# davelailai/DS-GCN

Hardware: AMD Instinct MI355X
Metric: clips/sec fwd+bwd, DS-STGCN NTU-60 3x64x25x2 (higher is better)
Workload: dtype f32; 1 GPU; DS-STGCN configs/dsstgcn/ntu60_xsub_3dkp/j.py (DSSTGCN_model.py kwargs), 64 clips/GPU of 3x64x25x2, 60 classes, train-mode BN, CE loss, fwd+bwd+grad all-reduce+SGD-nesterov per step; clips_per_gpu=64, global_batch=64, parallelism=dp1

## Files before the change

ds-gcn_amd/csrc/fuseout.hip:

```cpp
#include "common.h"
#include "dropout.h"
#include "dsgcn_jobs.h"

namespace {

__global__ __launch_bounds__(64) void k_fuse_out_fwd(const float* __restrict__ x1, const float* __restrict__ s1,
                                                     const float* __restrict__ h1, const float* __restrict__ x2,
                                                     const float* __restrict__ s2, const float* __restrict__ h2,
                                                     int relu, float* __restrict__ out, float* __restrict__ xbar, int C,
                                                     int T, int V, int vec, int ld, float* __restrict__ out_s2,
                                                     float* __restrict__ pmean, DropArgs dr) {
  extern __shared__ __attribute__((aligned(16))) float lds[];
  const int lane = threadIdx.x;
  const long plane = blockIdx.x;
  const int c = (int)(plane % C);
  const int L = T * V;
  const bool drop = dr.thresh != 0;
  const unsigned long long dstep = (drop && dr.step) ? (unsigned long long)*dr.step : 0ull;
  const float a1 = s1 ? s1[c] : 1.f, b1 = s1 ? h1[c] : 0.f;
  const float a2 = s2 ? s2[c] : 1.f, b2 = s2 ? h2[c] : 0.f;
  const float* p1 = x1 + (size_t)plane * L;
  const float* p2 = x2 ? x2 + (size_t)plane * L : nullptr;
  float* po = out ? out + (size_t)plane * L : nullptr;
  float psum = 0.f;
  if (vec) {
    const int L4 = L >> 2;
    const f32x4* q1 = reinterpret_cast<const f32x4*>(p1);
    const f32x4* q2 = reinterpret_cast<const f32x4*>(p2);
    f32x4* qo = reinterpret_cast<f32x4*>(po);
    f32x4* ql = reinterpret_cast<f32x4*>(lds);
#pragma unroll 4
    for (int i = lane; i < L4; i += 64) {
      f32x4 v = q1[i];
      v.x = fmaf(v.x, a1, b1); v.y = fmaf(v.y, a1, b1); v.z = fmaf(v.z, a1, b1); v.w = fmaf(v.w, a1, b1);
      if (relu & 2) { v.x = fmaxf(v.x, 0.f); v.y = fmaxf(v.y, 0.f); v.z = fmaxf(v.z, 0.f); v.w = fmaxf(v.w, 0.f); }
      if (drop) {
        unsigned rw[4];
        drop_words(dr, dstep, (unsigned long long)plane * L4 + i, rw);
        v.x *= rw[0] >= dr.thresh ? dr.inv : 0.f; v.y *= rw[1] >= dr.thresh ? dr.inv : 0.f;
        v.z *= rw[2] >= dr.thresh ? dr.inv : 0.f; v.w *= rw[3] >= dr.thresh ? dr.inv : 0.f;
      }
      if (p2) {
        const f32x4 r = q2[i];
        v.x += fmaf(r.x, a2, b2); v.y += fmaf(r.y, a2, b2); v.z += fmaf(r.z, a2, b2); v.w += fmaf(r.w, a2, b2);
      }
      if (relu & 1) { v.x = fmaxf(v.x, 0.f); v.y = fmaxf(v.y, 0.f); v.z = fmaxf(v.z, 0.f); v.w = fmaxf(v.w, 0.f); }
      if (po) qo[i] = v;
      psum += (v.x + v.y) + (v.z + v.w);
      if (xbar || out_s2) ql[i] = v;
    }
  } else {
    for (int i = lane; i < L; i += 64) {
      float v = fmaf(p1[i], a1, b1);
      if (relu & 2) v = fmaxf(v, 0.f);
      if (drop) v *= drop_mult(dr, dstep, (unsigned long long)plane * L + i);
      if (p2) v += fmaf(p2[i], a2, b2);
      if (relu & 1) v = fmaxf(v, 0.f);
      if (po) po[i] = v;
      psum += v;
      if (xbar || out_s2) lds[i] = v;
    }
  }
  if (pmean) {
    psum = wave_sum(psum);
    if (lane == 0) pmean[plane] = psum / (float)L;
  }
  if (xbar || out_s2) wave_lds_sync();
  if (out_s2) {
    const int T2 = (T + 1) >> 1, L2 = T2 * V;
    float* ps = out_s2 + (size_t)plane * L2;
    const float invV = 1.f / (float)V;
    if ((L2 & 3) == 0) {
      f32x4* q4 = reinterpret_cast<f32x4*>(ps);
      for (int i = lane; i < (L2 >> 2); i += 64) {
        int t, v;
        divmod_small(4 * i, V, invV, t, v);
        float r[4];
#pragma unroll
        for (int k = 0; k < 4; ++k) {
          r[k] = lds[2 * t * V + v];
          if (++v == V) { v = 0; ++t; }
        }
// ... 59 lines not shown
    float g = s3 == 3 ? gpl : (pg ? pg[i] : 0.f);
    if (pg2) g += pg2[i];
    if (pg3) {
      if (s3 == 2) { if (!(t & 1)) g += pg3[(t >> 1) * V + v]; }
      else g += pg3[i];
    }
    g += dxb[v];
    if ((relu & 1) && !(pre > 0.f)) g = 0.f;
    const float g1 = (((relu & 2) && !(pre1 > 0.f)) ? 0.f : g) * dm;
    o1[i] = g1 * a1;
    if (o2) o2[i] = g * a2;
    u0 = fmaf(g1, xa, u0);
    u1 += g;
    u2 = fmaf(g, xb, u2);
    u3 += g1;
    v += step;
    t += tstep;
    if (v >= V) { v -= V; ++t; }
  }
  if (part) {
    u0 = wave_sum(u0);
    u1 = wave_sum(u1);
    u2 = wave_sum(u2);
    u3 = wave_sum(u3);
    if (lane == 0) {
      part[(size_t)plane * 4 + 0] = u0;
      part[(size_t)plane * 4 + 1] = u1;
      part[(size_t)plane * 4 + 2] = u2;
      part[(size_t)plane * 4 + 3] = u3;
    }
  }
}

template <int NG, bool S3, bool X2>
__global__ __launch_bounds__(64) void k_fuse_out_bwd4(const float* __restrict__ x1, const float* __restrict__ s1,
                                                      const float* __restrict__ h1, const float* __restrict__ x2,
                                                      const float* __restrict__ s2, const float* __restrict__ h2,
                                                      int relu, const float* __restrict__ dout,
                                                      const float* __restrict__ dout2, const float* __restrict__ dout3,
                                                      const float* __restrict__ dxbar, float* __restrict__ dx1,
                                                      float* __restrict__ dx2, float* __restrict__ part, int C, int T,
                                                      int V, int ld, DropArgs dr) {
  __shared__ float dxb[32];
  const int lane = threadIdx.x;
  const long plane = blockIdx.x;
  const int c = (int)(plane % C);
  const int L = T * V, L4 = L >> 2;
  const bool drop = dr.thresh != 0;
  const unsigned long long dstep = (drop && dr.step) ? (unsigned long long)*dr.step : 0ull;
  const float a1 = s1 ? s1[c] : 1.f, b1 = s1 ? h1[c] : 0.f;
  const float a2 = s2 ? s2[c] : 1.f, b2 = s2 ? h2[c] : 0.f;
  if (lane < V) dxb[lane] = dxbar ? dxbar[(size_t)plane * ld + lane] / (float)T : 0.f;
  wave_lds_sync();
  const f32x4* __restrict__ p1 = reinterpret_cast<const f32x4*>(x1 + (size_t)plane * L);
  const f32x4* __restrict__ p2 = X2 ? reinterpret_cast<const f32x4*>(x2 + (size_t)plane * L) : nullptr;
  const f32x4* __restrict__ pg = NG >= 1 ? reinterpret_cast<const f32x4*>(dout + (size_t)plane * L) : nullptr;
  const float gplane = NG == 0 ? dout[plane] / (float)L : 0.f;
  const f32x4* __restrict__ pg2 = NG >= 2 ? reinterpret_cast<const f32x4*>(dout2 + (size_t)plane * L) : nullptr;
  const f32x4* __restrict__ pg3 = (NG >= 3 && !S3) ? reinterpret_cast<const f32x4*>(dout3 + (size_t)plane * L) : nullptr;
  const float* __restrict__ ps3 = S3 ? dout3 + (size_t)plane * (((T + 1) >> 1) * V) : nullptr;
  f32x4* __restrict__ o1 = reinterpret_cast<f32x4*>(dx1 + (size_t)plane * L);
  f32x4* __restrict__ o2 = X2 ? reinterpret_cast<f32x4*>(dx2 + (size_t)plane * L) : nullptr;
  const float invV = 1.f / (float)V;
  float u0 = 0.f, u1 = 0.f, u2 = 0.f, u3 = 0.f;
  for (int i = lane; i < L4; i += 64) {
    const f32x4 xa = p1[i];
    f32x4 xb = {0.f, 0.f, 0.f, 0.f}, g = {gplane, gplane, gplane, gplane};
    if constexpr (NG >= 1) g = pg[i];
    if constexpr (X2) xb = p2[i];
    if constexpr (NG >= 2) { const f32x4 w = pg2[i]; g.x += w.x; g.y += w.y; g.z += w.z; g.w += w.w; }
    if constexpr (NG >= 3 && !S3) { const f32x4 w = pg3[i]; g.x += w.x; g.y += w.y; g.z += w.z; g.w += w.w; }
    int t, v;
    divmod_small(4 * i, V, invV, t, v);
    f32x4 r1, r2;
    float dm[4] = {1.f, 1.f, 1.f, 1.f};
    if (drop) {
      unsigned rw[4];
      drop_words(dr, dstep, (unsigned long long)plane * L4 + i, rw);
#pragma unroll
      for (int k = 0; k < 4; ++k) dm[k] = rw[k] >= dr.thresh ? dr.inv : 0.f;
    }
#pragma unroll
    for (int k = 0; k < 4; ++k) {
      float gg = g[k];
      if constexpr (S3) { if (!(t & 1)) gg += ps3[(t >> 1) * V + v]; }
      gg += dxb[v];
      const float pre1 = fmaf(xa[k], a1, b1);
      float pre = ((relu & 2) ? fmaxf(pre1, 0.f) : pre1) * dm[k];
      if constexpr (X2) pre += fmaf(xb[k], a2, b2);
      if ((relu & 1) && !(pre > 0.f)) gg = 0.f;
      const float g1 = (((relu & 2) && !(pre1 > 0.f)) ? 0.f : gg) * dm[k];
      r1[k] = g1 * a1;
      r2[k] = gg * a2;
      u0 = fmaf(g1, xa[k], u0);
      u1 += gg;
      u2 = fmaf(gg, xb[k], u2);
      u3 += g1;
      if (++v == V) { v = 0; ++t; }
    }
    o1[i] = r1;
    if constexpr (X2) o2[i] = r2;
  }
  if (part) {
    u0 = wave_sum(u0);
    u1 = wave_sum(u1);
    u2 = wave_sum(u2);
    u3 = wave_sum(u3);
    if (lane == 0) {
      part[(size_t)plane * 4 + 0] = u0;
      part[(size_t)plane * 4 + 1] = u1;
      part[(size_t)plane * 4 + 2] = u2;
      part[(size_t)plane * 4 + 3] = u3;
    }
  }
}

int g_fo_vec = 1;

}

namespace {

DropArgs drop_args(const dsgcn_dropout* d) {
  DropArgs a = {};
  if (d && d->p > 0.f) {
    a.step = d->step; a.seed = d->seed; a.call = d->call;
    double t = (double)d->p * 4294967296.0;
    a.thresh = t >= 4294967295.0 ? 4294967295u : (t < 1.0 ? 1u : (unsigned)t);
    a.inv = 1.f / (1.f - d->p);
  }
  return a;
}

__global__ __launch_bounds__(256) void k_dropout_mask(float* __restrict__ mask, long numel, DropArgs dr) {
  const unsigned long long step = dr.step ? (unsigned long long)*dr.step : 0ull;
  for (long e = (long)blockIdx.x * 256 + threadIdx.x; e < numel; e += (long)gridDim.x * 256)
    mask[e] = dr.thresh ? drop_mult(dr, step, (unsigned long long)e) : 1.f;
}

}

extern "C" {

int dsgcn_fuse_out_fwd_drop(const float* x1, const float* s1, const float* h1, const float* x2, const float* s2,
                            const float* h2, int relu, float* out, float* out_s2, float* xbar, float* pmean, int n, int C,
                            int T, int V, int xbar_ld, const dsgcn_dropout* d, void* stream) {
  if (!x1 || (!out && !pmean) || n <= 0 || C <= 0 || T <= 0 || V <= 0 || V > 32 || (s1 && !h1) || (s2 && !h2)) return DSGCN_EINVAL;
  if ((out_s2 || xbar) && !out) return DSGCN_EINVAL;
  if (xbar && (xbar_ld < V || xbar_ld > 64)) return DSGCN_EINVAL;
  if (d && !(d->p >= 0.f && d->p < 1.f)) return DSGCN_EINVAL;
  const int vec = ((T * V) % 4 == 0) ? 1 : 0;
  const size_t lds = (xbar || out_s2) ? (size_t)T * V * sizeof(float) : 0;
  if (lds > 64 * 1024) return DSGCN_EUNSUPPORTED;
  hipLaunchKernelGGL(k_fuse_out_fwd, dim3((unsigned)((long)n * C)), dim3(64), lds, (hipStream_t)stream, x1, s1, h1, x2,
                     s2, h2, relu, out, xbar, C, T, V, vec, xbar ? xbar_ld : V, out_s2, pmean, drop_args(d));
  DSGCN_LAUNCH_CHECK();
  return 0;
}

int dsgcn_fuse_out_fwd(const float* x1, const float* s1, const float* h1, const float* x2, const float* s2,
                       const float* h2, int relu, float* out, float* xbar, int n, int C, int T, int V, int xbar_ld,
                       void* stream) {
  if (!out) return DSGCN_EINVAL;
  return dsgcn_fuse_out_fwd_drop(x1, s1, h1, x2, s2, h2, relu, out, nullptr, xbar, nullptr, n, C, T, V, xbar_ld, nullptr, stream);
}

int dsgcn_fuse_out_bwd_drop(const float* x1, const float* s1, const float* h1, const float* x2, const float* s2,
                            const float* h2, int relu, const float* dout, const float* dout2, const float* dout3,
                            int stride3, const float* dxbar, float* dx1, float* dx2, float* part, int n, int C, int T, int V,
                            int xbar_ld, const dsgcn_dropout* d, void* stream) {
  if (!x1 || !dx1 || n <= 0 || C <= 0 || T <= 0 || V <= 0 || V > 32 || (x2 && !dx2)) return DSGCN_EINVAL;
  if (dxbar && xbar_ld < V) return DSGCN_EINVAL;
  if ((dout2 || dout3) && !dout) return DSGCN_EINVAL;
  if (stride3 < 1 || stride3 > 3 || (stride3 == 3 && (!dout || dout2 || dout3 || dxbar))) return DSGCN_EINVAL;
  if (d && !(d->p >= 0.f && d->p < 1.f)) return DSGCN_EINVAL;
  const DropArgs dr = drop_args(d);
  const dim3 grid((unsigned)((long)n * C)), blk(64);
  hipStream_t st = (hipStream_t)stream;
  if (stride3 == 3) {
    if ((T * V) % 4 == 0) {
      if (x2)
        hipLaunchKernelGGL((k_fuse_out_bwd4<0, false, true>), grid, blk, 0, st, x1, s1, h1, x2, s2, h2, relu, dout,
                           (const float*)nullptr, (const float*)nullptr, (const float*)nullptr, dx1, dx2, part, C, T, V, V, dr);
      else
        hipLaunchKernelGGL((k_fuse_out_bwd4<0, false, false>), grid, blk, 0, st, x1, s1, h1, x2, s2, h2, relu, dout,
                           (const float*)nullptr, (const float*)nullptr, (const float*)nullptr, dx1, dx2, part, C, T, V, V, dr);
    } else {
      hipLaunchKernelGGL(k_fuse_out_bwd, grid, blk, 0, st, x1, s1, h1, x2, s2, h2, relu, dout, (const float*)nullptr,
                         (const float*)nullptr, (const float*)nullptr, dx1, dx2, part, C, T, V, V, 3, dr);
    }
    DSGCN_LAUNCH_CHECK();
    return 0;
  }
  if (g_fo_vec && dout && (T * V) % 4 == 0 && !(dout3 && !dout2 && stride3 == 1)) {
    const int ng = dout3 && stride3 == 1 ? 3 : (dout2 ? 2 : 1);
    const bool s3 = dout3 && stride3 == 2;
#define FO4(NGV, S3V, X2V) hipLaunchKernelGGL((k_fuse_out_bwd4<NGV, S3V, X2V>), grid, blk, 0, st, x1, s1, h1, x2, s2, h2, relu, \
                                              dout, dout2, dout3, dxbar, dx1, dx2, part, C, T, V, xbar_ld, dr)
    if (x2) {
      if (s3) { if (ng == 2) FO4(2, true, true); else FO4(1, true, true); }
      else if (ng == 3) FO4(3, false, true);
      else if (ng == 2) FO4(2, false, true);
      else FO4(1, false, true);
    } else {
      if (s3) { if (ng == 2) FO4(2, true, false); else FO4(1, true, false); }
      else if (ng == 3) FO4(3, false, false);
      else if (ng == 2) FO4(2, false, false);
      else FO4(1, false, false);
    }
#undef FO4
    DSGCN_LAUNCH_CHECK();
    return 0;
  }
  hipLaunchKernelGGL(k_fuse_out_bwd, grid, blk, 0, st, x1, s1, h1, x2, s2, h2, relu, dout, dout2, dout3, dxbar, dx1, dx2,
                     part, C, T, V, xbar_ld, stride3, dr);
  DSGCN_LAUNCH_CHECK();
  return 0;
}

int dsgcn_dropout_mask(float* mask, long numel, const dsgcn_dropout* d, void* stream) {
  if (!mask || numel <= 0 || (d && !(d->p >= 0.f && d->p < 1.f))) return DSGCN_EINVAL;
  const long blocks = (numel + 255) / 256;
  hipLaunchKernelGGL(k_dropout_mask, dim3((unsigned)(blocks > 4096 ? 4096 : blocks)), dim3(256), 0, (hipStream_t)stream, mask,
                     numel, drop_args(d));
  DSGCN_LAUNCH_CHECK();
  return 0;
}

#ifdef DSGCN_LAB
int dsgcn_fuse_out_tuning(int key, int value) {
  if (key != 0) return DSGCN_EINVAL;
  g_fo_vec = value;
  return 0;
}
#endif

int dsgcn_fuse_out_bwd(const float* x1, const float* s1, const float* h1, const float* x2, const float* s2,
                       const float* h2, int relu, const float* dout, const float* dxbar, float* dx1, float* dx2,
                       float* part, int n, int C, int T, int V, int xbar_ld, void* stream) {
  return dsgcn_fuse_out_bwd_drop(x1, s1, h1, x2, s2, h2, relu, dout, nullptr, nullptr, 1, dxbar, dx1, dx2, part, n, C, T, V,
                                 xbar_ld, nullptr, stream);
}

}

namespace {
__global__ __launch_bounds__(256) void k_pack(const float* const* __restrict__ src, const long* __restrict__ off,
                                              const int* __restrict__ numel, float* __restrict__ dst) {
  const int i = blockIdx.x;
  const float* __restrict__ s = src[i];
  float* __restrict__ d = dst + off[i];
  const int n = numel[i];
// ... 67 lines not shown
```

ds-gcn_amd/kernels.py:

```python
import contextlib
import sys

_active = None


def ops():
    return _active if _active is not None else sys.modules[__name__]


@contextlib.contextmanager
def use_ops(namespace):
    global _active
    prev = _active
    _active = namespace
    try:
        yield namespace
    finally:
        _active = prev


NAME = 'hip'

import torch

# ... 2350 lines not shown
FUSE_OUT_LDS_BYTES = 64 * 1024


def prestrided_fits(T, V):
    return T * V * 4 <= FUSE_OUT_LDS_BYTES


_drop_state = {'call': 0, 'step': {}, 'used': False}


def _dropout_record(p, device):
    st = _drop_state
    if device not in st['step']:
        st['step'][device] = torch.zeros((), dtype=torch.int64, device=device)
    st['call'] = (st['call'] + 1) & 0x7fffffff
    st['used'] = True
    step = st['step'][device]
    return native.Dropout(step.data_ptr(), int(torch.initial_seed()) & 0xffffffffffffffff, st['call'], float(p)), step


def dropout_step_advance():
    if _drop_state['used']:
        for step in _drop_state['step'].values():
            step.add_(1)


def dropout_mask(numel, rec):
    dev = next(iter(_drop_state['step']))
    out = torch.empty(numel, device=dev, dtype=torch.float32)
    native.check(native.lib().dsgcn_dropout_mask(_ptr(out), numel, _ct.byref(rec), _stream()), 'dsgcn_dropout_mask')
    return out


class _FuseOut(torch.autograd.Function):

    @staticmethod
    def forward(ctx, x1, s1, h1, x2, s2, h2, relu, xbar_ld, tee, dropout=0.0):
        _require_cuda(x1)
        x1, s1, h1, x2, s2, h2 = [_f32c(t) for t in (x1, s1, h1, x2, s2, h2)]
        n, C, T, V = x1.shape
        if x2 is not None and x2.shape != x1.shape:
            raise ValueError(f'fuse_out: the two terms differ in shape: {tuple(x1.shape)} vs {tuple(x2.shape)}')
        out = torch.empty_like(x1)
        out_s2 = torch.empty((n, C, (T + 1) // 2, V), device=x1.device, dtype=torch.float32) if tee == 2 else None
        xbar = torch.empty((n, C, xbar_ld), device=x1.device, dtype=torch.float32) if xbar_ld else None
        ctx.drop = _dropout_record(dropout, x1.device) if dropout > 0 else None
        rc = native.lib().dsgcn_fuse_out_fwd_drop(_ptr(x1), _ptr(s1), _ptr(h1), _ptr(x2), _ptr(s2), _ptr(h2), int(relu),
                                                  _ptr(out), _ptr(out_s2), _ptr(xbar), None, n, C, T, V, int(xbar_ld),
                                                  _ct.byref(ctx.drop[0]) if ctx.drop else None, _stream())
        native.check(rc, 'dsgcn_fuse_out_fwd_drop')
        ctx.save_for_backward(x1, s1, h1, x2, s2, h2)
        ctx.relu = int(relu)
        ctx.xbar_ld = int(xbar_ld)
        ctx.tee = int(tee)
        ctx.bn1, ctx.bn2 = _bn_of(s1), _bn_of(s2)
        ctx.set_materialize_grads(False)
        if tee == 2:
            return out, out.view_as(out), out_s2, xbar
        if tee:
            return out, out.view_as(out), out.view_as(out), xbar
        return out, None, None, xbar

    @staticmethod
    def backward(ctx, dout, dout2, dout3, dxbar):
        x1, s1, h1, x2, s2, h2 = ctx.saved_tensors
        n, C, T, V = x1.shape
        stride3 = 1
        for g, frames in ((dout, T), (dout2, T), (dout3, (T + 1) // 2 if ctx.tee == 2 else T)):
            if g is not None and tuple(g.shape) != (n, C, frames, V):
                raise ValueError(f'fuse_out backward: gradient of shape {tuple(g.shape)}, expected {(n, C, frames, V)}')
        if ctx.tee == 2:
            d3 = _f32c(dout3)
            full = [_f32c(g) for g in (dout, dout2) if g is not None]
            if d3 is not None and not full:
                full = [torch.zeros_like(x1)]
            douts = full + [None] * (2 - len(full)) + [d3]
            stride3 = 2 if d3 is not None else 1
        else:
            douts = [_f32c(g) for g in (dout, dout2, dout3) if g is not None]
            douts += [None] * (3 - len(douts))
        dxbar = _f32c(dxbar)
        dx1 = torch.empty_like(x1)
        dx2 = torch.empty_like(x2) if x2 is not None else None
        need_part = s1 is not None or s2 is not None
        part = torch.empty((n, C, 4), device=x1.device, dtype=torch.float32) if need_part else None
        rc = native.lib().dsgcn_fuse_out_bwd_drop(_ptr(x1), _ptr(s1), _ptr(h1), _ptr(x2), _ptr(s2), _ptr(h2), ctx.relu,
                                                  _ptr(douts[0]), _ptr(douts[1]), _ptr(douts[2]), stride3, _ptr(dxbar),
                                                  _ptr(dx1), _ptr(dx2), _ptr(part), n, C, T, V, ctx.xbar_ld or V,
                                                  _ct.byref(ctx.drop[0]) if ctx.drop else None, _stream())
        native.check(rc, 'dsgcn_fuse_out_bwd_drop')
        (ds1, dh1, ds2, dh2), _ = _affine_tail(part, 4, [(s1, ctx.bn1, 0, 3), (s2, ctx.bn2, 2, 1)])
        return dx1, ds1, dh1, dx2, ds2, dh2, None, None, None, None


class _FuseOutPool(torch.autograd.Function):

    @staticmethod
    def forward(ctx, x1, s1, h1, x2, s2, h2, relu, dropout=0.0):
        _require_cuda(x1)
        x1, s1, h1, x2, s2, h2 = [_f32c(t) for t in (x1, s1, h1, x2, s2, h2)]
        n, C, T, V = x1.shape
        if x2 is not None and x2.shape != x1.shape:
            raise ValueError(f'fuse_out_pool: the two terms differ in shape: {tuple(x1.shape)} vs {tuple(x2.shape)}')
        pm = torch.empty((n, C), device=x1.device, dtype=torch.float32)
        ctx.drop = _dropout_record(dropout, x1.device) if dropout > 0 else None
        rc = native.lib().dsgcn_fuse_out_fwd_drop(_ptr(x1), _ptr(s1), _ptr(h1), _ptr(x2), _ptr(s2), _ptr(h2), int(relu),
                                                  None, None, None, _ptr(pm), n, C, T, V, V,
                                                  _ct.byref(ctx.drop[0]) if ctx.drop else None, _stream())
        native.check(rc, 'dsgcn_fuse_out_fwd_drop')
        ctx.save_for_backward(x1, s1, h1, x2, s2, h2)
        ctx.relu = int(relu)
        ctx.bn1, ctx.bn2 = _bn_of(s1), _bn_of(s2)
        return pm

    @staticmethod
    def backward(ctx, dpm):
        x1, s1, h1, x2, s2, h2 = ctx.saved_tensors
        n, C, T, V = x1.shape
        dpm = _f32c(dpm)
        dx1 = torch.empty_like(x1)
        dx2 = torch.empty_like(x2) if x2 is not None else None
        need_part = s1 is not None or s2 is not None
        part = torch.empty((n, C, 4), device=x1.device, dtype=torch.float32) if need_part else None
# ... 164 lines not shown
```

ds-gcn_amd/native.py:

```python
import ctypes
import glob
import os
import subprocess

_HERE = os.path.dirname(os.path.abspath(__file__))
CSRC = os.path.join(_HERE, 'csrc')
LIB_DIR = os.path.join(_HERE, 'lib')
LIB_PATH = os.path.join(LIB_DIR, 'libdsgcn.so')
LAB_LIB_PATH = os.path.join(LIB_DIR, 'libdsgcn_lab.so')
INCLUDE = os.path.join(os.path.dirname(_HERE), 'include')

_lib = None
_lab = None
INITIAL_MATMUL_PRECISION = 0

c_f = ctypes.c_void_p
c_i = ctypes.c_void_p
c_int = ctypes.c_int
c_st = ctypes.c_void_p

SIGNATURES = {
    'dsgcn_version': [],
    'dsgcn_set_matmul_precision': [c_int],
    'dsgcn_get_matmul_precision': [],
# ... 73 lines not shown
    'dsgcn_ctr_affine_bwd': [ctypes.c_void_p, c_f, c_int, c_f, ctypes.c_void_p, c_f] + [c_int] * 4 + [c_st],
    'dsgcn_edge_select_fwd': [c_f, c_i, c_f] + [c_int] * 4 + [c_st],
    'dsgcn_edge_select_bwd': [c_f, c_i, c_f] + [c_int] * 4 + [c_st],
    'dsgcn_plane_stats': [c_f, c_f, ctypes.c_long, c_int, c_st],
    'dsgcn_typedconv_fwd': [c_f, c_f, c_f, c_i, c_int, c_f] + [c_int] * 7 + [c_st],
    'dsgcn_typedconv_dgrad': [c_f, c_f, c_i, c_int, c_f] + [c_int] * 7 + [c_st],
    'dsgcn_typedconv_wgrad_rows': [c_int] * 4,
    'dsgcn_typedconv_wgrad': [c_f, c_f, c_i, c_int, c_f] + [c_int] * 7 + [c_st],
    'dsgcn_add3': [c_f, c_f, c_f, c_f, ctypes.c_long, c_st],
    'dsgcn_pack': [c_f, c_f, c_f, c_int, c_f, c_st],
    'dsgcn_pack_fill': [c_f, c_f, c_f, c_int, c_f, c_st],
    'dsgcn_colsum_multi_host': [ctypes.c_void_p, c_int, c_st],
    'dsgcn_fuse_out_fwd': [c_f] * 6 + [c_int] + [c_f] * 2 + [c_int] * 5 + [c_st],
    'dsgcn_fuse_out_bwd': [c_f] * 6 + [c_int] + [c_f] * 5 + [c_int] * 5 + [c_st],
    'dsgcn_dwcausal_fwd': [c_f, c_f, c_f, c_i, c_f] + [c_int] * 6 + [c_st],
    'dsgcn_dwcausal_bwd': [c_f, c_f, c_i, c_f, c_f, c_f] + [c_int] * 6 + [c_st],
    'dsgcn_gate_fwd': [c_f, c_f, c_int, c_f, c_f] + [c_int] * 5 + [c_st],
    'dsgcn_gate_bwd': [c_f, c_f, c_int, c_f, c_f, c_int, c_f, c_f] + [c_int] * 4 + [c_st],
    'dsgcn_skeleton_prep': [ctypes.c_void_p] * 11 + [c_int] * 10 + [c_st],
    'dsgcn_skeleton_prep_streams': [ctypes.c_void_p] * 10 + [ctypes.POINTER(ctypes.c_void_p)] + [c_int] * 10 + [c_st],
    'dsgcn_dynadj_partial_stride': [c_int, c_int, c_int],
    'dsgcn_dynadj_supported': [c_int] * 6,
    'dsgcn_dynadj_fwd': [c_f] * 6 + [c_i, c_i, c_f] + [c_int] * 6 + [c_st],
    'dsgcn_dynadj_bwd': [c_f] * 5 + [c_i, c_i] + [c_f] * 4 + [c_int] * 7 + [c_st],
    'dsgcn_pwconv_group_ok': [c_int] * 5,
    'dsgcn_pwconv_fwd_group': [ctypes.c_void_p] * 3 + [c_int] + [ctypes.c_void_p] * 2 + [c_int] * 6 + [c_st],
    'dsgcn_pwconv_dgrad_group': [ctypes.c_void_p] * 3 + [c_int] + [ctypes.c_void_p] * 4 + [c_int] * 6 + [c_st],
    'dsgcn_pwconv_wgrad_group': [ctypes.c_void_p] * 3 + [c_int] + [ctypes.c_void_p] * 3 + [c_int] * 7 + [c_st],
    'dsgcn_pwconv_wgrad_jobs': [c_f] * 6 + [c_int] + [c_f] * 8 + [c_int] * 8 + [ctypes.c_void_p, c_int, c_st],
    'dsgcn_tms_split_wgrad_jobs': [c_f] * 4 + [c_int] + [c_f] * 2 + [c_int] * 6 + [c_i] * 4 + [ctypes.c_void_p, ctypes.c_void_p, c_int, c_int, ctypes.c_void_p, c_int, c_st],
    'dsgcn_fuse_out_fwd_drop': [c_f] * 6 + [c_int] + [c_f] * 4 + [c_int] * 5 + [ctypes.c_void_p, c_st],
    'dsgcn_fuse_out_bwd_drop': [c_f] * 6 + [c_int] + [c_f] * 3 + [c_int] + [c_f] * 4 + [c_int] * 5 + [ctypes.c_void_p, c_st],
    'dsgcn_dropout_mask': [c_f, ctypes.c_long, ctypes.c_void_p, c_st],
    'dsgcn_bn_finalize_multi': [ctypes.c_void_p, c_int, c_st],
    'dsgcn_bn_coef_rows_multi': [ctypes.c_void_p, c_int, c_st],
    'dsgcn_dyntyped_select_fwd': [c_f, c_i, c_f] + [c_int] * 5 + [c_st],
    'dsgcn_dyntyped_select_bwd': [c_f, c_i, c_f] + [c_int] * 5 + [c_st],
    'dsgcn_dyntyped_partial_stride': [c_int] * 4,
    'dsgcn_dyntyped_fwd': [c_f] * 6 + [c_i, c_f] + [c_int] * 5 + [c_st],
    'dsgcn_dyntyped_bwd': [c_f] * 5 + [c_i] + [c_f] * 5 + [c_int] * 6 + [c_st],
    'dsgcn_dynflag_partial_stride': [c_int] * 4,
    'dsgcn_dynflag_fwd': [c_f] * 8 + [c_i, c_i, c_f] + [c_int] * 7 + [c_st],
    'dsgcn_dynflag_bwd': [c_f] * 7 + [c_i, c_i] + [c_f] * 5 + [c_int] * 8 + [c_st],
    'dsgcn_dynplain_partial_stride': [c_int] * 2,
    'dsgcn_dynplain_fwd': [c_f] * 5 + [c_int] * 5 + [c_st],
    'dsgcn_dynplain_bwd': [c_f] * 6 + [c_int] * 6 + [c_st],
    'dsgcn_dynadj_fwd_jobs': [c_f] * 6 + [c_i, c_i, c_f] + [c_int] * 6 + [ctypes.c_void_p, c_int, c_st],
    'dsgcn_dynadj_bwd_jobs': [c_f] * 5 + [c_i, c_i] + [c_f] * 4 + [c_int] * 7 + [ctypes.c_void_p, c_int, c_st],
    'dsgcn_head_loss_fwd': [c_f, c_f, c_f, c_i] + [c_int] * 4 + [ctypes.c_float] + [c_f] * 6 + [c_st],
    'dsgcn_head_loss_bwd': [c_f, c_f, c_f, c_i, c_f] + [c_int] * 4 + [ctypes.c_float] + [c_f] * 3 + [c_st],
    'dsgcn_head_target_fwd': [c_f] * 4 + [ctypes.c_void_p] + [c_int] * 5 + [ctypes.c_float] + [c_f] * 7 + [c_st],
    'dsgcn_head_target_bwd': [c_f] * 5 + [c_int] * 4 + [ctypes.c_float] + [c_f] * 3 + [c_st],
    'dsgcn_head_test_fwd': [c_f, c_f, c_f] + [c_int] * 6 + [c_f, c_f, c_st],
    'dsgcn_head_ensemble_fwd': [ctypes.POINTER(ctypes.c_void_p)] * 3 + [c_f] + [c_int] * 7 + [c_f, c_f, c_st],
    'dsgcn_feat_ext_fwd': [c_f, c_f, c_f] + [c_int] * 8 + [c_f, ctypes.c_void_p, c_st],
    'dsgcn_data_bn_fwd': [c_f] * 10 + [c_int] * 7 + [ctypes.c_float, ctypes.c_float, c_st],
    'dsgcn_data_bn_bwd': [c_f] * 6 + [c_int] * 6 + [c_st],
    'dsgcn_sgd_step': [c_f, c_f, c_f, c_f, ctypes.c_float, ctypes.c_float, c_int, ctypes.c_longlong, c_st],
    'dsgcn_grad_norm_rows': [ctypes.c_longlong],
    'dsgcn_grad_norm_partials': [c_f, ctypes.c_longlong, c_int, ctypes.c_void_p, c_st],
    'dsgcn_sgd_step_clip': [c_f, c_f, c_f, c_f, ctypes.c_void_p, c_int, c_int, ctypes.c_float, c_f, ctypes.c_float,
                            ctypes.c_float, c_int, ctypes.c_longlong, c_st],
    'dsgcn_grad_accum': [c_f, c_f, ctypes.c_longlong, c_st],
    'dsgcn_grad_accum_finish': [c_f, c_f, c_f, ctypes.c_longlong, c_st],
    'dsgcn_optim_chunks': [ctypes.c_longlong],
    'dsgcn_optim_table': [ctypes.c_void_p, ctypes.c_void_p, c_int, ctypes.c_void_p, c_int, ctypes.c_longlong,
# ... 228 lines not shown
```

include/dsgcn.h:

```cpp
#ifndef DSGCN_H_
#define DSGCN_H_

#include <stddef.h>
#include "dsgcn_jobs.h"
#ifdef __cplusplus
extern "C" {
#endif

#define DSGCN_EINVAL (-1)
#define DSGCN_EUNSUPPORTED (-2)

int dsgcn_version(void);

int dsgcn_set_matmul_precision(int level);
int dsgcn_get_matmul_precision(void);
int dsgcn_pwconv_terms(int dir, int n, int Ci, int Co, int T, int V, int stride);
int dsgcn_tconv_terms(int dir, int n, int Ci, int Co, int T, int V, int KT, int stride);

int dsgcn_aggregate_fwd(const float* zp, const float* scale, const float* shift, int relu, const float* ahat,
                        float* y, int n, int KC, int T, int V, void* stream);

int dsgcn_aggregate_bwd_partial_rows(int n, int T, int V);
int dsgcn_aggregate_bwd(const float* zp, const float* scale, const float* shift, int relu, const float* ahat,
                        const float* dy, float* dzp, float* dahat, float* partial, int n, int KC, int T, int V,
// ... 26 lines not shown
int dsgcn_dyntyped_bwd(const float* x12, const float* pq, const float* be, const float* alpha, const float* beta,
                       const int* edge_type, const float* dahat, float* dd_ws, float* dx12, float* dpq, float* ppar,
                       int pstride, int n, int mid, int V, int E, int flags, void* stream);

int dsgcn_dynflag_partial_stride(int mid, int V, int E, int flags);
int dsgcn_dynflag_fwd(const float* proj, const float* pq, const float* be, const float* wa, const float* ba,
                      const float* A, const float* alpha, const float* beta, const int* node_type, const int* edge_type,
                      float* ahat, int n, int mid, int V, int ld, int P, int E, int flags, void* stream);
int dsgcn_dynflag_bwd(const float* proj, const float* pq, const float* be, const float* wa, const float* ba,
                      const float* alpha, const float* beta, const int* node_type, const int* edge_type,
                      const float* dahat, float* dd_ws, float* dproj, float* dpq, float* ppar, int pstride, int n,
                      int mid, int V, int ld, int P, int E, int flags, void* stream);

int dsgcn_dynplain_partial_stride(int K, int V);
int dsgcn_dynplain_fwd(const float* proj, const float* A, const float* alpha, const float* beta, float* ahat, int n, int K,
                       int mid, int V, int ld, void* stream);
int dsgcn_dynplain_bwd(const float* proj, const float* alpha, const float* beta, const float* dahat, float* dproj,
                       float* ppar, int pstride, int n, int K, int mid, int V, int ld, void* stream);

int dsgcn_fuse_out_fwd(const float* x1, const float* s1, const float* h1, const float* x2, const float* s2,
                       const float* h2, int relu, float* out, float* xbar, int n, int C, int T, int V, int xbar_ld,
                       void* stream);
int dsgcn_fuse_out_bwd(const float* x1, const float* s1, const float* h1, const float* x2, const float* s2,
                       const float* h2, int relu, const float* dout, const float* dxbar, float* dx1, float* dx2,
                       float* part, int n, int C, int T, int V, int xbar_ld, void* stream);
int dsgcn_fuse_out_fwd_drop(const float* x1, const float* s1, const float* h1, const float* x2, const float* s2,
                            const float* h2, int relu, float* out, float* out_s2, float* xbar, float* pmean, int n, int C,
                            int T, int V, int xbar_ld, const dsgcn_dropout* d, void* stream);
int dsgcn_fuse_out_bwd_drop(const float* x1, const float* s1, const float* h1, const float* x2, const float* s2,
                            const float* h2, int relu, const float* dout, const float* dout2, const float* dout3,
                            int stride3, const float* dxbar, float* dx1, float* dx2, float* part, int n, int C, int T, int V,
                            int xbar_ld, const dsgcn_dropout* d, void* stream);
int dsgcn_dropout_mask(float* mask, long numel, const dsgcn_dropout* d, void* stream);

size_t dsgcn_tconv_ws_bytes(int n, int Ci, int Co, int T, int V, int KT, int stride);
int dsgcn_tconv_wsplit(const float* w, int Ci, int Co, int KT, void* ws, void* stream);
int dsgcn_tconv_wsplit_multi(const dsgcn_tsplit_job* jobs, int njobs, void* stream);
int dsgcn_tconv_rows(int which, int n, int Ci, int Co, int T, int V, int KT, int stride);
int dsgcn_tconv_fwd(const float* x1, const float* s1, const float* h1, const float* x2, const float* s2, const float* h2,
                    int relu, const void* ws, const float* bias, float* z, float* partial, int n, int Ci, int Co, int T,
                    int V, int KT, int stride, void* stream);
int dsgcn_tconv_dgrad(const float* x1, const float* s1, const float* h1, const float* x2, const float* s2,
                      const float* h2, int relu, const void* ws, const float* z, const float* gz, const float* A0,
                      const float* B0, float* dx1, float* dx2, float* ipart, int n, int Ci, int Co, int T, int V, int KT,
                      int stride, void* stream);

int dsgcn_tconv_wgrad_splits(int n, int Ci, int Co, int T, int V, int KT, int stride);
int dsgcn_tconv_wgrad(const float* x1, const float* s1, const float* h1, const float* x2, const float* s2,
                      const float* h2, int relu, const float* z, const float* gz, const float* A0, const float* B0,
                      float* dwp, float* dbp, int pstride, int n, int Ci, int Co, int T, int V, int KT, int stride,
                      void* stream);

int dsgcn_branch_act_fwd(const float* z, const float* zaug, const float* scale, const float* shift, int n_act,
                         float* h, int n, int C, int T, int V, void* stream);
int dsgcn_branch_act_bwd(const float* z, const float* zaug, const float* scale, const float* shift, int n_act,
                         const float* dh, float* dz, float* dzaug, float* part, int n, int C, int T, int V,
                         void* stream);
int dsgcn_tapconv_fwd(const float* h, float* o, int n, int Cin, int Cout, int T, int V1, int stride, int KT, int nbr,
                      const int* type, const int* ci0, const int* co0, const int* cin, const int* cout, const int* dil,
                      const float* const* w, const float* const* b, void* stream);
int dsgcn_tapconv_dgrad(const float* h, const float* go, float* dh, int n, int Cin, int Cout, int T, int V1, int stride,
                        int KT, int nbr, const int* type, const int* ci0, const int* co0, const int* cin,
                        const int* cout, const int* dil, const float* const* w, void* stream);
int dsgcn_tapconv_wgrad_splits(int n, int Cin, int Cout, int T, int V1, int stride, int KT, int nbr, const int* type,
                               const int* cin, const int* cout, const int* dil);
int dsgcn_tapconv_wgrad(const float* h, const float* go, int n, int Cin, int Cout, int T, int V1, int stride, int KT,
// ... 274 lines not shown
```

Measured before the change: 6089 clips/s.

## Save a packed ReLU bitmask in fuse-out forward instead of reloading residual input

When the fused output has a residual term with no affine and a final ReLU, the forward kernel now packs the sign of each output element into a 1-bit mask. Backward reads that mask rather than the full float residual tensor x2 to recompute the ReLU gate, which cuts backward memory traffic for that kernel. The cost is an extra mask write plus wave shuffles in forward, and a small separate mask allocation. Keeping x2 saved for autograd does not by itself save memory. The path is on by default and can be disabled with an environment variable.

```diff
diff --git a/ds-gcn_amd/csrc/fuseout.hip b/ds-gcn_amd/csrc/fuseout.hip
--- a/ds-gcn_amd/csrc/fuseout.hip
+++ b/ds-gcn_amd/csrc/fuseout.hip
@@ -9,7 +9,8 @@
                                                      const float* __restrict__ s2, const float* __restrict__ h2,
                                                      int relu, float* __restrict__ out, float* __restrict__ xbar, int C,
                                                      int T, int V, int vec, int ld, float* __restrict__ out_s2,
-                                                     float* __restrict__ pmean, DropArgs dr) {
+                                                     float* __restrict__ pmean, DropArgs dr,
+                                                     unsigned* __restrict__ mask) {
   extern __shared__ __attribute__((aligned(16))) float lds[];
   const int lane = threadIdx.x;
   const long plane = blockIdx.x;
@@ -29,8 +30,7 @@
     const f32x4* q2 = reinterpret_cast<const f32x4*>(p2);
     f32x4* qo = reinterpret_cast<f32x4*>(po);
     f32x4* ql = reinterpret_cast<f32x4*>(lds);
-#pragma unroll 4
-    for (int i = lane; i < L4; i += 64) {
+    auto quad = [&](int i) -> f32x4 {
       f32x4 v = q1[i];
       v.x = fmaf(v.x, a1, b1); v.y = fmaf(v.y, a1, b1); v.z = fmaf(v.z, a1, b1); v.w = fmaf(v.w, a1, b1);
       if (relu & 2) { v.x = fmaxf(v.x, 0.f); v.y = fmaxf(v.y, 0.f); v.z = fmaxf(v.z, 0.f); v.w = fmaxf(v.w, 0.f); }
@@ -45,9 +45,33 @@
         v.x += fmaf(r.x, a2, b2); v.y += fmaf(r.y, a2, b2); v.z += fmaf(r.z, a2, b2); v.w += fmaf(r.w, a2, b2);
       }
       if (relu & 1) { v.x = fmaxf(v.x, 0.f); v.y = fmaxf(v.y, 0.f); v.z = fmaxf(v.z, 0.f); v.w = fmaxf(v.w, 0.f); }
-      if (po) qo[i] = v;
-      psum += (v.x + v.y) + (v.z + v.w);
-      if (xbar || out_s2) ql[i] = v;
+      return v;
+    };
+    if (mask) {
+      unsigned* __restrict__ pm = mask + (size_t)plane * ((L + 31) >> 5);
+      for (int base = 0; base < L4; base += 64) {
+        const int i = base + lane;
+        unsigned w = 0;
+        if (i < L4) {
+          const f32x4 v = quad(i);
+          w = ((v.x > 0.f ? 1u : 0u) | (v.y > 0.f ? 2u : 0u) | (v.z > 0.f ? 4u : 0u) | (v.w > 0.f ? 8u : 0u)) << ((lane & 7) * 4);
+          qo[i] = v;
+          psum += (v.x + v.y) + (v.z + v.w);
+          if (xbar || out_s2) ql[i] = v;
+        }
+        w |= __shfl_xor(w, 1, 64);
+        w |= __shfl_xor(w, 2, 64);
+        w |= __shfl_xor(w, 4, 64);
+        if ((lane & 7) == 0 && i < L4) pm[i >> 3] = w;
+      }
+    } else {
+#pragma unroll 4
+      for (int i = lane; i < L4; i += 64) {
+        const f32x4 v = quad(i);
+        if (po) qo[i] = v;
+        psum += (v.x + v.y) + (v.z + v.w);
+        if (xbar || out_s2) ql[i] = v;
+      }
     }
   } else {
     for (int i = lane; i < L; i += 64) {
@@ -173,15 +197,17 @@
   }
 }
 
-template <int NG, bool S3, bool X2>
-__global__ __launch_bounds__(64) void k_fuse_out_bwd4(const float* __restrict__ x1, const float* __restrict__ s1,
-                                                      const float* __restrict__ h1, const float* __restrict__ x2,
-                                                      const float* __restrict__ s2, const float* __restrict__ h2,
-                                                      int relu, const float* __restrict__ dout,
-                                                      const float* __restrict__ dout2, const float* __restrict__ dout3,
-                                                      const float* __restrict__ dxbar, float* __restrict__ dx1,
-                                                      float* __restrict__ dx2, float* __restrict__ part, int C, int T,
-                                                      int V, int ld, DropArgs dr) {
+template <int NG, bool S3, bool X2, bool MASK>
+__device__ __forceinline__ void fuse_out_bwd4_body(const float* __restrict__ x1, const float* __restrict__ s1,
+                                                   const float* __restrict__ h1, const float* __restrict__ x2,
+                                                   const unsigned* __restrict__ mask,
+                                                   const float* __restrict__ s2, const float* __restrict__ h2,
+                                                   int relu, const float* __restrict__ dout,
+                                                   const float* __restrict__ dout2, const float* __restrict__ dout3,
+                                                   const float* __restrict__ dxbar, float* __restrict__ dx1,
+                                                   float* __restrict__ dx2, float* __restrict__ part, int C, int T,
+                                                   int V, int ld, DropArgs dr) {
+  static_assert(!MASK || X2, "the mask stands in for a second term");
   __shared__ float dxb[32];
   const int lane = threadIdx.x;
   const long plane = blockIdx.x;
@@ -194,7 +220,8 @@
   if (lane < V) dxb[lane] = dxbar ? dxbar[(size_t)plane * ld + lane] / (float)T : 0.f;
   wave_lds_sync();
   const f32x4* __restrict__ p1 = reinterpret_cast<const f32x4*>(x1 + (size_t)plane * L);
-  const f32x4* __restrict__ p2 = X2 ? reinterpret_cast<const f32x4*>(x2 + (size_t)plane * L) : nullptr;
+  const f32x4* __restrict__ p2 = (X2 && !MASK) ? reinterpret_cast<const f32x4*>(x2 + (size_t)plane * L) : nullptr;
+  const unsigned* __restrict__ pm = MASK ? mask + (size_t)plane * ((L + 31) >> 5) : nullptr;
   const f32x4* __restrict__ pg = NG >= 1 ? reinterpret_cast<const f32x4*>(dout + (size_t)plane * L) : nullptr;
   const float gplane = NG == 0 ? dout[plane] / (float)L : 0.f;
   const f32x4* __restrict__ pg2 = NG >= 2 ? reinterpret_cast<const f32x4*>(dout2 + (size_t)plane * L) : nullptr;
@@ -208,7 +235,9 @@
     const f32x4 xa = p1[i];
     f32x4 xb = {0.f, 0.f, 0.f, 0.f}, g = {gplane, gplane, gplane, gplane};
     if constexpr (NG >= 1) g = pg[i];
-    if constexpr (X2) xb = p2[i];
+    if constexpr (X2 && !MASK) xb = p2[i];
+    unsigned bits = 0;
+    if constexpr (MASK) bits = pm[i >> 3] >> ((i & 7) * 4);
     if constexpr (NG >= 2) { const f32x4 w = pg2[i]; g.x += w.x; g.y += w.y; g.z += w.z; g.w += w.w; }
     if constexpr (NG >= 3 && !S3) { const f32x4 w = pg3[i]; g.x += w.x; g.y += w.y; g.z += w.z; g.w += w.w; }
     int t, v;
@@ -227,15 +256,19 @@
       if constexpr (S3) { if (!(t & 1)) gg += ps3[(t >> 1) * V + v]; }
       gg += dxb[v];
       const float pre1 = fmaf(xa[k], a1, b1);
-      float pre = ((relu & 2) ? fmaxf(pre1, 0.f) : pre1) * dm[k];
-      if constexpr (X2) pre += fmaf(xb[k], a2, b2);
-      if ((relu & 1) && !(pre > 0.f)) gg = 0.f;
+      if constexpr (MASK) {
+        if ((relu & 1) && !((bits >> k) & 1u)) gg = 0.f;
+      } else {
+        float pre = ((relu & 2) ? fmaxf(pre1, 0.f) : pre1) * dm[k];
+        if constexpr (X2) pre += fmaf(xb[k], a2, b2);
+        if ((relu & 1) && !(pre > 0.f)) gg = 0.f;
+      }
       const float g1 = (((relu & 2) && !(pre1 > 0.f)) ? 0.f : gg) * dm[k];
       r1[k] = g1 * a1;
       r2[k] = gg * a2;
       u0 = fmaf(g1, xa[k], u0);
       u1 += gg;
-      u2 = fmaf(gg, xb[k], u2);
+      if constexpr (!MASK) u2 = fmaf(gg, xb[k], u2);
       u3 += g1;
       if (++v == V) { v = 0; ++t; }
     }
@@ -256,6 +289,31 @@
   }
 }
 
+template <int NG, bool S3, bool X2>
+__global__ __launch_bounds__(64) void k_fuse_out_bwd4(const float* __restrict__ x1, const float* __restrict__ s1,
+                                                      const float* __restrict__ h1, const float* __restrict__ x2,
+                                                      const float* __restrict__ s2, const float* __restrict__ h2,
+                                                      int relu, const float* __restrict__ dout,
+                                                      const float* __restrict__ dout2, const float* __restrict__ dout3,
+                                                      const float* __restrict__ dxbar, float* __restrict__ dx1,
+                                                      float* __restrict__ dx2, float* __restrict__ part, int C, int T,
+                                                      int V, int ld, DropArgs dr) {
+  fuse_out_bwd4_body<NG, S3, X2, false>(x1, s1, h1, x2, nullptr, s2, h2, relu, dout, dout2, dout3, dxbar, dx1, dx2, part, C,
+                                        T, V, ld, dr);
+}
+
+template <int NG, bool S3>
+__global__ __launch_bounds__(64) void k_fuse_out_bwd4m(const float* __restrict__ x1, const float* __restrict__ s1,
+                                                       const float* __restrict__ h1, const unsigned* __restrict__ mask,
+                                                       int relu, const float* __restrict__ dout,
+                                                       const float* __restrict__ dout2, const float* __restrict__ dout3,
+                                                       const float* __restrict__ dxbar, float* __restrict__ dx1,
+                                                       float* __restrict__ dx2, float* __restrict__ part, int C, int T,
+                                                       int V, int ld, DropArgs dr) {
+  fuse_out_bwd4_body<NG, S3, true, true>(x1, s1, h1, nullptr, mask, nullptr, nullptr, relu, dout, dout2, dout3, dxbar, dx1,
+                                         dx2, part, C, T, V, ld, dr);
+}
+
 int g_fo_vec = 1;
 
 }
@@ -279,24 +337,38 @@
     mask[e] = dr.thresh ? drop_mult(dr, step, (unsigned long long)e) : 1.f;
 }
 
-}
-
-extern "C" {
-
-int dsgcn_fuse_out_fwd_drop(const float* x1, const float* s1, const float* h1, const float* x2, const float* s2,
-                            const float* h2, int relu, float* out, float* out_s2, float* xbar, float* pmean, int n, int C,
-                            int T, int V, int xbar_ld, const dsgcn_dropout* d, void* stream) {
+int fuse_out_fwd_launch(const float* x1, const float* s1, const float* h1, const float* x2, const float* s2,
+                        const float* h2, int relu, float* out, float* out_s2, float* xbar, float* pmean, unsigned* mask,
+                        int n, int C, int T, int V, int xbar_ld, const dsgcn_dropout* d, void* stream) {
   if (!x1 || (!out && !pmean) || n <= 0 || C <= 0 || T <= 0 || V <= 0 || V > 32 || (s1 && !h1) || (s2 && !h2)) return DSGCN_EINVAL;
   if ((out_s2 || xbar) && !out) return DSGCN_EINVAL;
   if (xbar && (xbar_ld < V || xbar_ld > 64)) return DSGCN_EINVAL;
   if (d && !(d->p >= 0.f && d->p < 1.f)) return DSGCN_EINVAL;
   const int vec = ((T * V) % 4 == 0) ? 1 : 0;
+  if (mask && !vec) return DSGCN_EUNSUPPORTED;
   const size_t lds = (xbar || out_s2) ? (size_t)T * V * sizeof(float) : 0;
   if (lds > 64 * 1024) return DSGCN_EUNSUPPORTED;
   hipLaunchKernelGGL(k_fuse_out_fwd, dim3((unsigned)((long)n * C)), dim3(64), lds, (hipStream_t)stream, x1, s1, h1, x2,
-                     s2, h2, relu, out, xbar, C, T, V, vec, xbar ? xbar_ld : V, out_s2, pmean, drop_args(d));
-  DSGCN_LAUNCH_CHECK();
-  return 0;
+                     s2, h2, relu, out, xbar, C, T, V, vec, xbar ? xbar_ld : V, out_s2, pmean, drop_args(d), mask);
+  DSGCN_LAUNCH_CHECK();
+  return 0;
+}
+
+}
+
+extern "C" {
+
+int dsgcn_fuse_out_fwd_drop(const float* x1, const float* s1, const float* h1, const float* x2, const float* s2,
+                            const float* h2, int relu, float* out, float* out_s2, float* xbar, float* pmean, int n, int C,
+                            int T, int V, int xbar_ld, const dsgcn_dropout* d, void* stream) {
+  return fuse_out_fwd_launch(x1, s1, h1, x2, s2, h2, relu, out, out_s2, xbar, pmean, nullptr, n, C, T, V, xbar_ld, d, stream);
+}
+
+int dsgcn_fuse_out_fwd_mask(const float* x1, const float* s1, const float* h1, const float* x2, const float* s2,
+                            const float* h2, int relu, float* out, float* out_s2, float* xbar, float* pmean, unsigned* mask,
+                            int n, int C, int T, int V, int xbar_ld, const dsgcn_dropout* d, void* stream) {
+  if (!mask || !out || !(relu & 1)) return DSGCN_EINVAL;
+  return fuse_out_fwd_launch(x1, s1, h1, x2, s2, h2, relu, out, out_s2, xbar, pmean, mask, n, C, T, V, xbar_ld, d, stream);
 }
 
 int dsgcn_fuse_out_fwd(const float* x1, const float* s1, const float* h1, const float* x2, const float* s2,
@@ -359,6 +431,32 @@
   return 0;
 }
 
+int dsgcn_fuse_out_bwd_mask(const float* x1, const float* s1, const float* h1, const unsigned* mask, const float* s2,
+                            const float* h2, int relu, const float* dout, const float* dout2, const float* dout3,
+                            int stride3, const float* dxbar, float* dx1, float* dx2, float* part, int n, int C, int T, int V,
+                            int xbar_ld, const dsgcn_dropout* d, void* stream) {
+  if (!x1 || !mask || !dx1 || !dx2 || !dout || n <= 0 || C <= 0 || T <= 0 || V <= 0 || V > 32) return DSGCN_EINVAL;
+  if (s2 || h2 || !(relu & 1) || (s1 && !h1)) return DSGCN_EINVAL;
+  if (dxbar && xbar_ld < V) return DSGCN_EINVAL;
+  if (stride3 < 1 || stride3 > 2 || (dout3 && !dout2 && stride3 == 1)) return DSGCN_EINVAL;
+  if (d && !(d->p >= 0.f && d->p < 1.f)) return DSGCN_EINVAL;
+  if ((T * V) % 4 != 0) return DSGCN_EUNSUPPORTED;
+  const DropArgs dr = drop_args(d);
+  const dim3 grid((unsigned)((long)n * C)), blk(64);
+  hipStream_t st = (hipStream_t)stream;
+  const int ng = dout3 && stride3 == 1 ? 3 : (dout2 ? 2 : 1);
+  const bool s3 = dout3 && stride3 == 2;
+#define FO4M(NGV, S3V) hipLaunchKernelGGL((k_fuse_out_bwd4m<NGV, S3V>), grid, blk, 0, st, x1, s1, h1, mask, relu, dout, dout2, \
+                                          dout3, dxbar, dx1, dx2, part, C, T, V, xbar_ld, dr)
+  if (s3) { if (ng == 2) FO4M(2, true); else FO4M(1, true); }
+  else if (ng == 3) FO4M(3, false);
+  else if (ng == 2) FO4M(2, false);
+  else FO4M(1, false);
+#undef FO4M
+  DSGCN_LAUNCH_CHECK();
+  return 0;
+}
+
 int dsgcn_dropout_mask(float* mask, long numel, const dsgcn_dropout* d, void* stream) {
   if (!mask || numel <= 0 || (d && !(d->p >= 0.f && d->p < 1.f))) return DSGCN_EINVAL;
   const long blocks = (numel + 255) / 256;
diff --git a/ds-gcn_amd/kernels.py b/ds-gcn_amd/kernels.py
--- a/ds-gcn_amd/kernels.py
+++ b/ds-gcn_amd/kernels.py
@@ -2406,6 +2406,10 @@
     return out
 
 
+RELU_BITS = _os.environ.get('DSGCN_RELU_BITS', '1') != '0'
+RELU_BITS_COUNTS = dict(fwd=0, bwd=0)
+
+
 class _FuseOut(torch.autograd.Function):
 
     @staticmethod
@@ -2419,11 +2423,21 @@
         out_s2 = torch.empty((n, C, (T + 1) // 2, V), device=x1.device, dtype=torch.float32) if tee == 2 else None
         xbar = torch.empty((n, C, xbar_ld), device=x1.device, dtype=torch.float32) if xbar_ld else None
         ctx.drop = _dropout_record(dropout, x1.device) if dropout > 0 else None
-        rc = native.lib().dsgcn_fuse_out_fwd_drop(_ptr(x1), _ptr(s1), _ptr(h1), _ptr(x2), _ptr(s2), _ptr(h2), int(relu),
-                                                  _ptr(out), _ptr(out_s2), _ptr(xbar), None, n, C, T, V, int(xbar_ld),
-                                                  _ct.byref(ctx.drop[0]) if ctx.drop else None, _stream())
-        native.check(rc, 'dsgcn_fuse_out_fwd_drop')
-        ctx.save_for_backward(x1, s1, h1, x2, s2, h2)
+        mask = None
+        if (RELU_BITS and x2 is not None and s2 is None and (int(relu) & 1) and (T * V) % 4 == 0
+                and any(ctx.needs_input_grad)):
+            mask = torch.empty((n, C, (T * V + 31) // 32), device=x1.device, dtype=torch.int32)
+            rc = native.lib().dsgcn_fuse_out_fwd_mask(_ptr(x1), _ptr(s1), _ptr(h1), _ptr(x2), None, None, int(relu),
+                                                      _ptr(out), _ptr(out_s2), _ptr(xbar), None, _ptr(mask), n, C, T, V,
+                                                      int(xbar_ld), _ct.byref(ctx.drop[0]) if ctx.drop else None, _stream())
+            native.check(rc, 'dsgcn_fuse_out_fwd_mask')
+            RELU_BITS_COUNTS['fwd'] += 1
+        else:
+            rc = native.lib().dsgcn_fuse_out_fwd_drop(_ptr(x1), _ptr(s1), _ptr(h1), _ptr(x2), _ptr(s2), _ptr(h2), int(relu),
+                                                      _ptr(out), _ptr(out_s2), _ptr(xbar), None, n, C, T, V, int(xbar_ld),
+                                                      _ct.byref(ctx.drop[0]) if ctx.drop else None, _stream())
+            native.check(rc, 'dsgcn_fuse_out_fwd_drop')
+        ctx.save_for_backward(x1, s1, h1, x2, s2, h2, mask)
         ctx.relu = int(relu)
         ctx.xbar_ld = int(xbar_ld)
         ctx.tee = int(tee)
@@ -2437,7 +2451,7 @@
 
     @staticmethod
     def backward(ctx, dout, dout2, dout3, dxbar):
-        x1, s1, h1, x2, s2, h2 = ctx.saved_tensors
+        x1, s1, h1, x2, s2, h2, mask = ctx.saved_tensors
         n, C, T, V = x1.shape
         stride3 = 1
         for g, frames in ((dout, T), (dout2, T), (dout3, (T + 1) // 2 if ctx.tee == 2 else T)):
@@ -2458,11 +2472,19 @@
         dx2 = torch.empty_like(x2) if x2 is not None else None
         need_part = s1 is not None or s2 is not None
         part = torch.empty((n, C, 4), device=x1.device, dtype=torch.float32) if need_part else None
-        rc = native.lib().dsgcn_fuse_out_bwd_drop(_ptr(x1), _ptr(s1), _ptr(h1), _ptr(x2), _ptr(s2), _ptr(h2), ctx.relu,
-                                                  _ptr(douts[0]), _ptr(douts[1]), _ptr(douts[2]), stride3, _ptr(dxbar),
-                                                  _ptr(dx1), _ptr(dx2), _ptr(part), n, C, T, V, ctx.xbar_ld or V,
-                                                  _ct.byref(ctx.drop[0]) if ctx.drop else None, _stream())
-        native.check(rc, 'dsgcn_fuse_out_bwd_drop')
+        if mask is not None and douts[0] is not None:
+            rc = native.lib().dsgcn_fuse_out_bwd_mask(_ptr(x1), _ptr(s1), _ptr(h1), _ptr(mask), None, None, ctx.relu,
+                                                      _ptr(douts[0]), _ptr(douts[1]), _ptr(douts[2]), stride3, _ptr(dxbar),
+                                                      _ptr(dx1), _ptr(dx2), _ptr(part), n, C, T, V, ctx.xbar_ld or V,
+                                                      _ct.byref(ctx.drop[0]) if ctx.drop else None, _stream())
+            native.check(rc, 'dsgcn_fuse_out_bwd_mask')
+            RELU_BITS_COUNTS['bwd'] += 1
+        else:
+            rc = native.lib().dsgcn_fuse_out_bwd_drop(_ptr(x1), _ptr(s1), _ptr(h1), _ptr(x2), _ptr(s2), _ptr(h2), ctx.relu,
+                                                      _ptr(douts[0]), _ptr(douts[1]), _ptr(douts[2]), stride3, _ptr(dxbar),
+                                                      _ptr(dx1), _ptr(dx2), _ptr(part), n, C, T, V, ctx.xbar_ld or V,
+                                                      _ct.byref(ctx.drop[0]) if ctx.drop else None, _stream())
+            native.check(rc, 'dsgcn_fuse_out_bwd_drop')
         (ds1, dh1, ds2, dh2), _ = _affine_tail(part, 4, [(s1, ctx.bn1, 0, 3), (s2, ctx.bn2, 2, 1)])
         return dx1, ds1, dh1, dx2, ds2, dh2, None, None, None, None
 
diff --git a/ds-gcn_amd/native.py b/ds-gcn_amd/native.py
--- a/ds-gcn_amd/native.py
+++ b/ds-gcn_amd/native.py
@@ -129,6 +129,9 @@
     'dsgcn_fuse_out_fwd_drop': [c_f] * 6 + [c_int] + [c_f] * 4 + [c_int] * 5 + [ctypes.c_void_p, c_st],
     'dsgcn_fuse_out_bwd_drop': [c_f] * 6 + [c_int] + [c_f] * 3 + [c_int] + [c_f] * 4 + [c_int] * 5 + [ctypes.c_void_p, c_st],
     'dsgcn_dropout_mask': [c_f, ctypes.c_long, ctypes.c_void_p, c_st],
+    'dsgcn_fuse_out_fwd_mask': [c_f] * 6 + [c_int] + [c_f] * 4 + [ctypes.c_void_p] + [c_int] * 5 + [ctypes.c_void_p, c_st],
+    'dsgcn_fuse_out_bwd_mask': [c_f] * 3 + [ctypes.c_void_p] + [c_f] * 2 + [c_int] + [c_f] * 3 + [c_int] + [c_f] * 4 +
+                               [c_int] * 5 + [ctypes.c_void_p, c_st],
     'dsgcn_bn_finalize_multi': [ctypes.c_void_p, c_int, c_st],
     'dsgcn_bn_coef_rows_multi': [ctypes.c_void_p, c_int, c_st],
     'dsgcn_dyntyped_select_fwd': [c_f, c_i, c_f] + [c_int] * 5 + [c_st],
diff --git a/include/dsgcn.h b/include/dsgcn.h
--- a/include/dsgcn.h
+++ b/include/dsgcn.h
@@ -82,6 +82,13 @@
                             int stride3, const float* dxbar, float* dx1, float* dx2, float* part, int n, int C, int T, int V,
                             int xbar_ld, const dsgcn_dropout* d, void* stream);
 int dsgcn_dropout_mask(float* mask, long numel, const dsgcn_dropout* d, void* stream);
+int dsgcn_fuse_out_fwd_mask(const float* x1, const float* s1, const float* h1, const float* x2, const float* s2,
+                            const float* h2, int relu, float* out, float* out_s2, float* xbar, float* pmean, unsigned* mask,
+                            int n, int C, int T, int V, int xbar_ld, const dsgcn_dropout* d, void* stream);
+int dsgcn_fuse_out_bwd_mask(const float* x1, const float* s1, const float* h1, const unsigned* mask, const float* s2,
+                            const float* h2, int relu, const float* dout, const float* dout2, const float* dout3,
+                            int stride3, const float* dxbar, float* dx1, float* dx2, float* part, int n, int C, int T, int V,
+                            int xbar_ld, const dsgcn_dropout* d, void* stream);
 
 size_t dsgcn_tconv_ws_bytes(int n, int Ci, int Co, int T, int V, int KT, int stride);
 int dsgcn_tconv_wsplit(const float* w, int Ci, int Co, int KT, void* ws, void* stream);
```

Result: no change. 6127 clips/s (median of 6 runs) (+0.6%).
